# codebits1001/CET-driven-simulation-for-3D-printing-AM-KMC-Approach

Measured on AMD Instinct MI355X. Metric: kmc_events_per_sec, higher is better.
Workload: dtype f64

## Files before the change

cet-driven-simulation-for-3d-printing-am-kmc-approach_amd/cetkmc/_lib.py:

```python
import ctypes as C
import glob
import os
import subprocess

_HERE = os.path.dirname(os.path.abspath(__file__))
CSRC = os.path.join(os.path.dirname(_HERE), "csrc")
INCLUDE = os.path.join(os.path.dirname(os.path.dirname(_HERE)), "include")
SO_PATH = os.path.join(CSRC, "libcetkmc_hip.so")


def sources():
    return sorted(glob.glob(os.path.join(CSRC, "*.hip")) + glob.glob(os.path.join(CSRC, "*.hpp")) +
                  glob.glob(os.path.join(INCLUDE, "*.h")))


HIPCC_FLAGS = ["--offload-arch=gfx950", "-O3", "-std=c++17", "-fPIC", "-shared", "-ffp-contract=off",
               "-fno-fast-math", "-I/opt/rocm/include"]


class Params(C.Structure):
    _fields_ = [
        ("nu", C.c_double), ("nu_dep", C.c_double), ("E_b", C.c_double * 3), ("E_diff", C.c_double * 3),
        ("kT", C.c_double), ("T_melt", C.c_double), ("I0", C.c_double), ("delta_T_c", C.c_double),
        ("K_nuc", C.c_double), ("beta_imp_nuc", C.c_double), ("max_imp_frac", C.c_double),
# ... 20 lines not shown
        ("np_cap", C.c_int64), ("rng_mode", C.c_int32), ("seed", C.c_uint64), ("thermal_mode", C.c_int32),
        ("thermal_dt", C.c_double), ("q_planes", C.POINTER(C.c_double)), ("n_q", C.c_int64),
        ("use_latent", C.c_int32), ("profile", C.c_int32), ("incremental", C.c_int32),
    ]


class SuperArgs(C.Structure):
    _fields_ = [
        ("step0", C.c_int64), ("n_steps", C.c_int64), ("box", C.c_int32), ("defect_fraction", C.c_double),
        ("seed", C.c_uint64), ("thermal_mode", C.c_int32), ("thermal_dt", C.c_double),
        ("q_planes", C.POINTER(C.c_double)), ("n_q", C.c_int64), ("use_latent", C.c_int32), ("null_events", C.c_int32),
    ]


class LocalArgs(C.Structure):
    _fields_ = [
        ("step0", C.c_int64), ("n_steps", C.c_int64), ("box", C.c_int32), ("defect_fraction", C.c_double),
        ("seed", C.c_uint64), ("thermal_mode", C.c_int32), ("thermal_dt", C.c_double), ("max_events", C.c_int32),
        ("horizon_events", C.c_double),
    ]


class LaneTableInfo(C.Structure):
    _fields_ = [(n, C.c_int64) for n in ("fresh", "chunks", "usable", "poisoned", "builds")]


class Counters(C.Structure):
    _fields_ = [(n, C.c_int64) for n in ("steps", "sweeps", "incremental_steps", "thermal_updates", "supersteps", "bytes_h2d",
                                         "bytes_d2h", "alg_bytes_sweep", "alg_bytes_thermal", "profiled_steps")] + \
               [(n, C.c_double) for n in ("ms_thermal", "ms_interface", "ms_sweep", "ms_dirty_rows", "ms_reduce", "ms_select_apply")] + \
               [(n, C.c_int64) for n in ("alg_bytes_table", "table_updates", "interface_launches")] + \
               [("ms_comm", C.c_double), ("comm_calls", C.c_int64), ("deferred_steps", C.c_int64),
                ("early_tiles", C.c_int64)]


ALLGATHER_FN = C.CFUNCTYPE(C.c_int, C.c_void_p, C.c_void_p, C.c_void_p, C.c_int64)
EXCHANGE_FN = C.CFUNCTYPE(C.c_int, C.c_void_p, C.c_int, C.c_int, C.c_void_p, C.c_void_p, C.c_void_p, C.c_void_p, C.c_int64)


class HostComm(C.Structure):
    _fields_ = [("allgather", ALLGATHER_FN), ("exchange", EXCHANGE_FN), ("user", C.c_void_p)]


class RunResult(C.Structure):
    _fields_ = [
        ("steps_done", C.c_int64), ("status", C.c_int32), ("np_used", C.c_int64), ("q_used", C.c_int64),
        ("nucleation_count", C.c_int64), ("sweep_ms_total", C.c_double), ("sweep_launches", C.c_int64),
# ... 97 lines not shown
STRUCT_MIRRORS = {"params": Params, "event": Event, "sweep_info": SweepInfo, "run_args": RunArgs, "run_result": RunResult,
                  "super_args": SuperArgs, "counters": Counters, "host_comm": HostComm, "ens_args": EnsArgs,
                  "ens_analysis": EnsAnalysis, "front_stats": FrontStats, "layer_rec": LayerRec,
                  "texture_args": TextureArgs, "grain_rec": GrainRec, "solid_info": SolidInfo, "solid_args": SolidArgs,
                  "solid_rec": SolidRec, "origin_rec": OriginRec, "local_args": LocalArgs,
                  "remelt_info": RemeltInfo, "substep_info": SubstepInfo, "implicit_info": ImplicitInfo,
                  "thermal_boundary": ThermalBoundary, "boundary_info": BoundaryInfo,
                  "beam": Beam, "beam_info": BeamInfo}

_P = C.POINTER
PROTOTYPES = {
    "cetkmc_last_error": (C.c_char_p, []),
    "cetkmc_abi_version": (C.c_int, []),
    "cetkmc_source_hash": (C.c_char_p, []),
    "cetkmc_struct_size": (C.c_int, [C.c_char_p]),
    "cetkmc_dirty_offset": (C.c_int, [C.c_int, C.c_int]),
    "cetkmc_stale_row": (C.c_int, [C.c_int, _P(C.c_int), _P(C.c_int), C.c_int, C.c_int]),
    "cetkmc_stale_rows": (C.c_int, [C.c_int, _P(C.c_int), _P(C.c_int), C.c_int, C.c_void_p]),
    "cetkmc_table_tile_of": (C.c_int, [C.c_int, C.c_int, C.c_int]),
    "cetkmc_early_tile_row": (C.c_int, [C.c_int, C.c_int, C.c_int, C.c_int]),
    "cetkmc_lane_needs_values": (C.c_int, [C.c_uint64]),
    "cetkmc_lane_request": (C.c_int, [C.c_uint64, C.c_int]),
    "cetkmc_lane_table": (C.c_int, [C.c_void_p, _P(LaneTableInfo)]),
    "cetkmc_invalidates": (C.c_int, [C.c_char_p]),
    "cetkmc_device_count": (C.c_int, [_P(C.c_int)]),
    "cetkmc_create": (C.c_int, [_P(Params), C.c_int, C.c_int, _P(C.c_int), _P(C.c_void_p)]),
    "cetkmc_get_unique_id": (C.c_int, [C.c_char_p]),
    "cetkmc_create_rank": (C.c_int, [_P(Params), C.c_int, C.c_int, C.c_int, C.c_int, C.c_char_p, _P(C.c_void_p)]),
    "cetkmc_create_rank_host": (C.c_int, [_P(Params), C.c_int, C.c_int, C.c_int, C.c_int, _P(HostComm), _P(C.c_void_p)]),
    "cetkmc_destroy": (C.c_int, [C.c_void_p]),
    "cetkmc_set_params": (C.c_int, [C.c_void_p, _P(Params)]),
    "cetkmc_sync": (C.c_int, [C.c_void_p]),
    "cetkmc_set_option": (C.c_int, [C.c_void_p, C.c_char_p, C.c_int64]),
    "cetkmc_owned_planes": (C.c_int, [C.c_void_p, _P(C.c_int), _P(C.c_int)]),
    "cetkmc_upload": (C.c_int, [C.c_void_p, C.c_void_p, C.c_void_p, C.c_void_p, C.c_void_p, C.c_void_p]),
    "cetkmc_download": (C.c_int, [C.c_void_p, C.c_void_p, C.c_void_p, C.c_void_p, C.c_void_p, C.c_void_p]),
    "cetkmc_upload_planes": (C.c_int, [C.c_void_p, C.c_int, C.c_int, C.c_void_p, C.c_void_p, C.c_void_p, C.c_void_p, C.c_void_p]),
    "cetkmc_download_planes": (C.c_int, [C.c_void_p, C.c_int, C.c_int, C.c_void_p, C.c_void_p, C.c_void_p, C.c_void_p, C.c_void_p]),
    "cetkmc_set_defects": (C.c_int, [C.c_void_p, C.c_void_p]),
    "cetkmc_set_prev_state": (C.c_int, [C.c_void_p, C.c_void_p]),
    "cetkmc_thermal_cet": (C.c_int, [C.c_void_p, C.c_double, C.c_int]),
    "cetkmc_thermal_laser": (C.c_int, [C.c_void_p, C.c_double, C.c_void_p, C.c_int, C.c_int]),
    "cetkmc_rate_sweep": (C.c_int, [C.c_void_p, _P(SweepInfo)]),
    "cetkmc_select": (C.c_int, [C.c_void_p, C.c_double, _P(Event)]),
    "cetkmc_apply": (C.c_int, [C.c_void_p, _P(Event), C.c_double, C.c_double, C.c_int]),
    "cetkmc_enumerate_events": (C.c_int, [C.c_void_p, C.c_void_p, C.c_int64, _P(C.c_int64)]),
# ... 169 lines not shown
```

cet-driven-simulation-for-3d-printing-am-kmc-approach_amd/cetkmc/engine.py:

```python
import ctypes as C

import numpy as np

from . import _lib
from ._lib import Counters, EnsAnalysis, EnsArgs, Event, LaneTableInfo, LocalArgs, Params, RunArgs, RunResult, SuperArgs, SweepInfo, build_library

EVENT_DTYPE = np.dtype([("type", "<i4"), ("pos", "<i4", 3), ("target", "<i4", 3), ("atom", "<i4"),
                        ("rate", "<f8"), ("dep_rank", "<i8"), ("theta", "<f8"), ("phi", "<f8")], align=True)
assert EVENT_DTYPE.itemsize == C.sizeof(Event) == 64
FRONT_DTYPE = np.dtype([("n_front", "<i8"), ("n_skipped", "<i8"), ("pos_sum", "<i8", 3), ("G_sum", "<f8"), ("G_min", "<f8"),
                        ("G_max", "<f8"), ("Gi_sum", "<f8"), ("T_sum", "<f8"), ("n_melt", "<i8"), ("melt_bbox", "<i4", 6)],
                       align=True)
assert FRONT_DTYPE.itemsize == C.sizeof(_lib.FrontStats) == 112
LAYER_DTYPE = np.dtype([("n_occ", "<i8"), ("n_start", "<i8"), ("n_eq", "<i8"), ("seg", "<i8", 3), ("cut", "<i8", 3),
                        ("occ_state", "<i8", 4), ("gb_state", "<i8", 4), ("pad", "<i8")])
assert LAYER_DTYPE.itemsize == C.sizeof(_lib.LayerRec) == 144
GRAIN_DTYPE = np.dtype([("n", "<i8"), ("sum", "<i8", 3), ("sq", "<i8", 6), ("n_state", "<i8", 4), ("nb", "<i8", 4),
                        ("first_theta", "<f8"), ("first_phi", "<f8")])
assert GRAIN_DTYPE.itemsize == C.sizeof(_lib.GrainRec) == 160
SOLID_DTYPE = np.dtype([("n_rec", "<i8"), ("n_bad", "<i8"), ("n_cooling", "<i8"), ("stamp_sum", "<i8"), ("stamp_min", "<i8"),
                        ("stamp_max", "<i8"), ("q", "<i8", 4)])
assert SOLID_DTYPE.itemsize == C.sizeof(_lib.SolidRec) == 80
SOLID_INFO_DTYPE = np.dtype([("n_new", "<i8"), ("n_cleared", "<i8"), ("n_recorded", "<i8")])
assert SOLID_INFO_DTYPE.itemsize == C.sizeof(_lib.SolidInfo) == 24
# ... 431 lines not shown
        res = RunResult()
        totals = np.zeros(n + 1, np.float64) if want_logs else None
        events = np.zeros(max(n, 1), dtype=EVENT_DTYPE) if want_logs else None
        nev = np.zeros(max(n, 1), np.int64) if want_logs else None
        self._ck(self.lib.cetkmc_run_steps(self.h, C.byref(a), C.byref(res), _ptr(totals), _ptr(events), _ptr(nev)))
        done = res.steps_done
        out = dict(done=int(done), status=int(res.status), np_used=int(res.np_used), q_used=int(res.q_used),
                   nucleation_count=int(res.nucleation_count), sweep_ms_total=res.sweep_ms_total,
                   sweep_launches=int(res.sweep_launches), wall_ms=res.wall_ms, full_sweeps=int(res.full_sweeps),
                   min_margin=float(res.min_margin))
        if want_logs:
            out.update(totals=totals[:done + (1 if res.status == 1 else 0)], events=events[:done], n_events=nev[:done])
        return out

    def counters(self, reset=False):
        c = Counters()
        self._ck(self.lib.cetkmc_get_counters(self.h, C.byref(c), int(bool(reset))))
        return {n: getattr(c, n) for n, _ in Counters._fields_}

    def lane_table(self):
        info = LaneTableInfo()
        self._ck(self.lib.cetkmc_lane_table(self.h, C.byref(info)))
        return {n: int(getattr(info, n)) for n, _ in LaneTableInfo._fields_}

    def run_supersteps(self, step0, n, box, defect_fraction, seed, thermal_mode=1, thermal_dt=1e-6, q_planes=None,
                       use_latent=True, want_events=False, null_events=False):
        a = SuperArgs()
        q = None if q_planes is None else np.ascontiguousarray(q_planes, dtype=np.float64)
        a.step0, a.n_steps, a.box, a.defect_fraction, a.seed = int(step0), int(n), int(box), float(defect_fraction), int(seed)
        a.thermal_mode, a.thermal_dt = int(thermal_mode), float(thermal_dt)
        a.q_planes, a.n_q, a.use_latent = _dptr(q), (0 if q is None else q.shape[0]), int(bool(use_latent))
        a.null_events = int(bool(null_events))
        nbx = self.L // int(box) if box and self.L % int(box) == 0 else 1
        D = max(1, (self.i1 - self.i0) // int(box)) * nbx * nbx if box and self.L % int(box) == 0 else 1
        return self._supersteps(self.lib.cetkmc_run_supersteps, a, n, D, (D,) if want_events else None)

    def _supersteps(self, call, a, n, D, event_shape, more=()):
        res = RunResult()
        totals = np.zeros(n + 1, np.float64)
        n_exec = np.zeros(max(n, 1), np.int64)
        dt_event = np.zeros(max(n, 1), np.float64)
        events = None if event_shape is None else np.zeros((max(n, 1),) + event_shape, dtype=EVENT_DTYPE)
        logs = {name: np.zeros(max(n, 1), dtype) for name, dtype in more}
        self._ck(call(self.h, C.byref(a), C.byref(res), _ptr(totals), _ptr(events), _ptr(n_exec), _ptr(dt_event),
                      *[_ptr(v) for v in logs.values()]))
        done = int(res.steps_done)
# ... 495 lines not shown
```

cet-driven-simulation-for-3d-printing-am-kmc-approach_amd/csrc/cetkmc_hip.hip:

```cpp
#include <dlfcn.h>
#include <hip/hip_runtime.h>
#include <hip/hip_ext.h>
#include <rccl/rccl.h>

#include <algorithm>
#include <chrono>
#include <cmath>
#include <cstdint>
#include <climits>
#include <cstdio>
#include <cstring>
#include <map>
#include <mutex>
#include <string>
#include <type_traits>
#include <vector>

#include "kernels.hpp"
#include "cluster.hpp"
#include "superstep.hpp"
#include "local.hpp"
#include "ensemble.hpp"
#include "front.hpp"
#include "layer.hpp"
// ... 125 lines not shown
    KParams kp{};
    int L = 0, Pk = 1, PB = 1, RJ = 0, pitchS = 0, pitchT = 0, pitchC = 0;
    int dev = 0;
    hipStream_t stream = nullptr, stream2 = nullptr;
    std::vector<Slab> slabs;
    SlabView* d_views[4] = {nullptr, nullptr, nullptr, nullptr};
    int cur = 0;
    int row_par = 0;
    int G = 1, my_first = 0;
    int own_i0 = 0, own_i1 = 0;
    BlockEnt* d_blocks = nullptr;
    cetkmc_event* d_events_all = nullptr;
    StepState* d_ss = nullptr;
    int* d_dirty = nullptr;
    PendRec* d_pend = nullptr;
    int apply_in_sweep = 1;
    int fused_tiles = 1;
    int table_lane_skip = 1;
    int lane_sums = 1;
    int early_tiles = -1;
    int early_blocks = 256;
    int poison_alt_rows = 0;
    bool pend_live = false;
    int64_t cnt_lane_builds = 0;
    int pend_early = 0;
    BatchCfg pend_cfg{};
    double* d_ktab = nullptr;
    KParams* d_kp = nullptr;
    void* d_scratch = nullptr;
    size_t scratch_bytes = 0;
    int* d_flag = nullptr;
    double* d_qtop = nullptr;
    double *d_u_pick = nullptr, *d_u_defect = nullptr, *d_u_np = nullptr, *d_q = nullptr, *d_log_total = nullptr;
    cetkmc_event* d_log_event = nullptr;
    int64_t* d_log_nev = nullptr;
    size_t cap_steps = 0, cap_np = 0, cap_q = 0;
    char* pin_in = nullptr; size_t pin_in_cap = 0;
    char* pin_out = nullptr; size_t pin_out_cap = 0;
    struct { bool valid = false, has_defect = false; int64_t step0 = 0, n_steps = 0, np_cap = 0, n_q = 0; int thermal_mode = 0; } staged;
    ncclComm_t comm = nullptr;
    int rank = 0, nranks = 1;
    bool swept = false;
    int sweep_auto = 1;
    int sweep_variant = 1;
    bool table_fresh = false;
    bool ifc_fresh = false;
    bool lanes_fresh = false;
// ... 504 lines not shown
    h->table_fresh = true;
    invalidate(h, Cause::table_written);
    return 0;
}

StreamArgs stream_args(Handle* h, const SlabView& v)
{
    StreamArgs sa{};
    sa.T_melt = h->kp.T_melt; sa.delta_T_c = h->kp.delta_T_c; sa.kT = h->kp.kT; sa.I0 = h->kp.I0;
    sa.rate_threshold = h->kp.rate_threshold; sa.K0 = host_k_eff(h->p, 0, 0);
    sa.L = v.L; sa.gi0 = v.gi0; sa.nloc = v.nloc; sa.RJ = v.RJ; sa.pitchC = v.pitchC; sa.pitchT = v.pitchT; sa.Pk = v.Pk;
    sa.cls = v.cls; sa.T = v.T; sa.vval = v.vval; sa.dep_val = v.dep_val; sa.rowsum = v.rowsum; sa.rowcnt = v.rowcnt;
    sa.lanesum = v.lanesum; sa.lanecnt = v.lanecnt;
    sa.group_first = 0; sa.group_count = (v.nloc + STREAM_NI - 1) / STREAM_NI;
    return sa;
}

TableCfg table_cfg(Handle* h, const Slab& s, int par)
{
    TableCfg tb{};
    tb.T_melt = h->kp.T_melt; tb.delta_T_c = h->kp.delta_T_c; tb.kT = h->kp.kT; tb.I0 = h->kp.I0;
    tb.rate_threshold = h->kp.rate_threshold; tb.K0 = host_k_eff(h->p, 0, 0); tb.nu_dep = h->kp.nu_dep;
    tb.vval = s.vvalbuf[par]; tb.dep_val = s.depbuf[par];
    return tb;
}

int refresh_ifc_grid(Handle* h)
{
    for (auto& sl : h->slabs) {
        int n_list = 0;
        HIPCHK(hipMemcpy(&n_list, sl.v.ifc_n, sizeof(int), hipMemcpyDeviceToHost));
        grow_ifc_grid(h, n_list);
    }
    return 0;
}

inline bool multi_rank(const Handle* h) { return h->comm != nullptr || h->hc.allgather != nullptr; }
int one_slab_only(const Handle* h, const std::string& who, const char* why)
{
    if (h->slabs.size() != 1 || h->nranks != 1 || multi_rank(h)) return fail(who + " needs the whole lattice in one slab of one process" + why);
    return 0;
}
int thermal_exclusions(const ThermalSettings& s, const char* fn)
{
    const struct { bool on; const char *what, *setter, *mode_b, *ahead; } rows[] = {
        {s.remelt_on != 0, "remelting is on", "cetkmc_set_remelt", "Mode B has no melt", "the field computed ahead knows no melt"},
// ... 102 lines not shown
        if (sv == 4) {
            with_rows(rs, [&](auto hw, auto ch2) {
                launch(k_sweep_plane<hw.value, ch2.value>, dim3((unsigned)v.nloc), dim3(1024), plane_shmem(h->L), h->stream, xa, xb, sa, ss, h->d_blocks);
            });
        } else if (sv == 3) {
            const int ipp = rs.hw ? (h->L + 1) / 2 : h->L;
            const int64_t n_items = (int64_t)ipp * v.nloc;
            const dim3 g((unsigned)((n_items + 4 * TABLE_IPW - 1) / (4 * TABLE_IPW)));
            with_rows(rs, [&](auto hw, auto ch2) {
                launch(k_sweep_table<hw.value, ch2.value>, g, dim3(256), 0, h->stream, xa, xb, sa, ss);
            });
        } else if (h->sweep_variant >= 1 && h->pend_live) {
            ApplyArgs X{h->kp, (const SlabView*)dviews(h), h->d_pend, h->d_ss, h->pend_cfg, (const double*)h->d_u_defect,
                        (const double*)h->d_u_np, (const double*)h->d_ktab, h->d_log_total, h->d_log_event, h->d_log_nev};
            if (table_tiles(h, 1))
                with_flag(h->table_lane_skip != 0, [&](auto ls) {
                    with_flag(lane_table_use(h), [&](auto lu) {
                        const int late = table_tile_count(h->L, v.nloc, true) - h->pend_early;
                        launch(k_sweep_stream_apply<true, 1, false, true, ls.value, ls.value && lu.value>, dim3(late + 1), dim3(256), apply_shmem(), h->stream, xa, xb, sa, h->d_ss, X, h->pend_early);
                    });
                });
            else
                launch(k_sweep_stream_apply<true, 1, false>, dim3(sa.group_count * njt + 1), dim3(256), h->shmem_stream, h->stream, xa, xb, sa, h->d_ss, X, 0);
        } else if (h->sweep_variant == 1 && table_tiles(h, 2)) {
            const bool build = lane_table_on(h) && !h->lanes_fresh;
            with_flag(h->table_lane_skip != 0, [&](auto ls) {
                with_flag(build, [&](auto lb) {
                    launch(k_sweep_stream<true, true, 1, false, true, ls.value, lb.value>, dim3(table_tile_count(h->L, v.nloc, true)), dim3(256), 0, h->stream, xa, xb, sa, ss);
                });
            });
            if (build) { h->lanes_fresh = true; ++h->cnt_lane_builds; }
        } else if (h->sweep_variant >= 1) {
            auto go = [&](auto k) { launch(k, dim3(sa.group_count * njt), dim3(256), h->shmem_stream, h->stream, xa, xb, sa, ss); };
            if (h->sweep_variant == 1 && lane_table_on(h) && !h->lanes_fresh) {
                go(k_sweep_stream<true, true, 1, false, false, false, true>);
                h->lanes_fresh = true; ++h->cnt_lane_builds;
            }
            else if (h->sweep_variant == 1) with_stream_kernel<true>(rs, go); else with_stream_kernel<false>(rs, go);
        } else {
            hipLaunchKernelGGL(k_sweep_simple, dim3(v.nloc * njt), dim3(256), shmem0, h->stream, h->kp, v, h->d_ktab, ss);
        }
    }
    if (ev_b && !ext) HIPCHK(hipEventRecord(ev_b, h->stream));
    if (sv != 4)
        for (size_t s = 0; s < h->slabs.size(); ++s) {
            SlabView v = view_of(h, (int)s);
// ... 119 lines not shown
    if (multi_rank(h) && h->nranks > 1) {
        Slab& s = h->slabs[0];
        double* T = s.Tbuf[buf];
        CHK(comm_exchange(h, T + plane * 2, T, T + plane * s.v.nloc, T + plane * (s.v.nloc + 2), 2 * plane * 8));
    }
    return 0;
}

ThermalCfg thermal_cfg(Handle* h, double dt, int laser, int use_latent, int scrub)
{
    ThermalCfg C{};
    C.dt = dt; C.alpha = h->p.alpha; C.inv_dx2 = h->p.inv_dx2; C.clip_lo = h->p.T_clip_lo; C.clip_hi = h->p.T_clip_hi;
    C.T_nan = h->p.T_nan; C.rho_cp = h->p.rho_cp; C.latent_coef = h->p.latent_coef;
    C.laser = laser; C.use_latent = use_latent; C.scrub = scrub; C.ni = h->therm_ni;
    return C;
}

int launch_thermal_one(Handle* h, double dt, int laser, const double* d_q, int use_latent, int scrub, bool batch, bool first = true)
{
    const ThermalCfg C = thermal_cfg(h, dt, laser, use_latent, scrub);
    if (first) ++h->cnt.thermal_updates;
    for (auto& sl : h->slabs) h->cnt.alg_bytes_thermal += (int64_t)16 * sl.v.nloc * h->L * h->L;
    const int nxt = h->cur ^ 1;
    size_t n_fused = 0;
    const StepState* ssp = batch ? h->d_ss : nullptr;
    for (size_t s = 0; s < h->slabs.size(); ++s) {
        SlabView v = view_of(h, (int)s);
        const double* Tin = h->slabs[s].Tbuf[h->cur];
        double* Tout = h->slabs[s].Tbuf[nxt];
        uint8_t* prev = h->slabs[s].prev;
        if (h->thermal_variant == 1) {
            const dim3 grid = thermal_grid(h->L, v.nloc, h->therm_ni);
            if (h->L % THERM_KT == 0 && h->L % THERM16_TJ == 0 && !h->thermal_general && h->thermal_tiles16) {
                ThermalCfg C16 = C;
                C16.ni = h->therm_ni16;
                const dim3 g16(h->L / h->thermal_kt, h->L / THERM16_TJ, (v.nloc + C16.ni - 1) / C16.ni);
                const bool fuse = h->thermal_table && h->thermal_rpt == 2 && h->thermal_kt == 256 && h->sweep_variant >= 1;
                if (fuse) { ++n_fused; h->cnt.alg_bytes_table += (int64_t)8 * v.nloc * v.L * v.L; }
                with_source(laser, use_latent, [&](auto la, auto lt) {
                    auto go = [&](auto k, unsigned threads, const TableCfg& tb) {
                        launch(k, g16, dim3(threads), 0, h->stream, nullptr, nullptr, v, Tin, Tout, prev, d_q, C16, ssp, tb);
                    };
                    if (fuse) go(k_thermal_tiles16<la.value, lt.value, 2, 256, true>, 1024, table_cfg(h, h->slabs[s], nxt));
                    else if (h->thermal_rpt == 2 && h->thermal_kt == 128) go(k_thermal_tiles16<la.value, lt.value, 2, 128>, 512, TableCfg{});
                    else if (h->thermal_rpt == 2) go(k_thermal_tiles16<la.value, lt.value, 2, 256>, 1024, TableCfg{});
                    else go(k_thermal_tiles16<la.value, lt.value, 4, 256>, 512, TableCfg{});
                });
            } else if (h->L % THERM_KT == 0 && h->L % THERM_TJ == 0 && !h->thermal_general) {
                with_source(laser, use_latent, [&](auto la, auto lt) {
                    launch(k_thermal_tiles<la.value, lt.value>, grid, dim3(256), 0, h->stream, nullptr, nullptr, v, Tin, Tout, prev, d_q, C, ssp);
                });
            } else {
                hipLaunchKernelGGL(k_thermal_march, grid, dim3(256), 0, h->stream, v, Tin, Tout, prev, d_q, C, ssp);
            }
        } else {
            hipLaunchKernelGGL(k_thermal, dim3((h->L + 255) / 256, h->L, v.nloc), dim3(256), 0, h->stream, v, Tin, Tout,
                               (const uint8_t*)prev, d_q, C, ssp);
        }
    }
    HIPCHK(hipGetLastError());
    CHK(exchange_T_halo(h, nxt));
    if (laser && use_latent) {
        for (auto& s : h->slabs) {
            if (h->thermal_variant != 1)
                HIPCHK(hipMemcpyAsync(s.prev, s.v.state, s.nS, hipMemcpyDeviceToDevice, h->stream));
            hipLaunchKernelGGL(k_clear_row_flags, dim3(64), dim3(256), 0, h->stream, s.v, batch ? (const StepState*)h->d_ss : nullptr);
        }
        HIPCHK(hipGetLastError());
    }
    h->cur = nxt;
    const bool wrote_table = n_fused == h->slabs.size();
    invalidate(h, wrote_table ? Cause::thermal_update_wrote_table : Cause::thermal_update);
    if (wrote_table) { h->table_fresh = true; ++h->cnt.table_updates; }
    return 0;
}

int substep_block_of(const Handle* h)
{
    if (h->slabs.size() != 1 || multi_rank(h) || h->thermal_variant != 1) return 1;
    if (h->substep_block) return h->substep_block;
    return h->L > SUB_PLAIN_L ? SUB_SDEFAULT : 1;
}
int substep_planes_of(Handle* h, int S)
{
    if (h->substep_planes) return h->substep_planes;
    if (!h->n_cu && hipDeviceGetAttribute(&h->n_cu, hipDeviceAttributeMultiprocessorCount, h->dev) != hipSuccess) { (void)hipGetLastError(); h->n_cu = 256; }
    const int tiles = ((h->L + SUB_EK - 2 * S - 1) / (SUB_EK - 2 * S)) * ((h->L + SUB_EJ - 2 * S - 1) / (SUB_EJ - 2 * S));
    const int groups = std::max(1, h->n_cu / tiles), nloc = h->slabs[0].v.nloc;
    return std::max((nloc + groups - 1) / groups, std::min(nloc, 8));
}
template <int LASER, int S>
void launch_sub_S(Handle* h, const SlabView& v, const double* Tin, double* Tout, const double* d_q, const ThermalCfg& C, const StepState* ssp)
{
    const dim3 grid((h->L + SUB_EK - 2 * S - 1) / (SUB_EK - 2 * S), (h->L + SUB_EJ - 2 * S - 1) / (SUB_EJ - 2 * S), (v.nloc + C.ni - 1) / C.ni);
    launch(k_thermal_sub<LASER, S>, grid, dim3(SUB_THREADS), 0, h->stream, nullptr, nullptr, v, Tin, Tout, d_q, C, ssp);
}
// ... 563 lines not shown
    se.type = type; se.pi = pos[0]; se.pj = pos[1]; se.ti = target[0]; se.tj = target[1];
    return se;
}
int cetkmc_stale_row(int type, const int pos[2], const int target[2], int gi, int j)
{
    return stale_row(stale_ev_host(type, pos, target), gi, j) ? 1 : 0;
}
int cetkmc_lane_needs_values(uint64_t class8)
{
    return lane_needs_values(make_uint2((unsigned)class8, (unsigned)(class8 >> 32))) ? 1 : 0;
}
int cetkmc_lane_request(uint64_t class8, int count_byte)
{
    static_assert(LANE_REQ_NONE == CETKMC_LANE_REQ_NONE && LANE_REQ_VALUES == CETKMC_LANE_REQ_VALUES && LANE_REQ_SUM == CETKMC_LANE_REQ_SUM, "cetkmc.h");
    return lane_request(make_uint2((unsigned)class8, (unsigned)(class8 >> 32)), (unsigned)count_byte & 0xFFu);
}
int cetkmc_lane_table(void* handle, cetkmc_lane_table_info* out)
{
    Handle* h = (Handle*)handle;
    if (!h || !out) return fail("null argument");
    *out = cetkmc_lane_table_info{};
    out->fresh = lane_table_use(h) ? 1 : 0;
    out->builds = h->cnt_lane_builds;
    if (h->slabs.size() != 1 || !h->slabs[0].v.lanecnt) return 0;
    HIPCHK(hipSetDevice(h->dev));
    CHK(ensure_scratch(h, 2 * sizeof(unsigned long long)));
    unsigned long long* d = (unsigned long long*)h->d_scratch;
    unsigned long long got[2] = {0, 0};
    HIPCHK(hipMemsetAsync(d, 0, sizeof got, h->stream));
    hipLaunchKernelGGL(k_lane_census, dim3(256), dim3(256), 0, h->stream, h->slabs[0].v, d);
    HIPCHK(hipGetLastError());
    HIPCHK(hipMemcpyAsync(got, d, sizeof got, hipMemcpyDeviceToHost, h->stream));
    HIPCHK(hipStreamSynchronize(h->stream));
    out->chunks = (int64_t)h->slabs[0].v.nloc * h->L * (h->pitchT / 8);
    out->usable = (int64_t)got[0];
    out->poisoned = (int64_t)got[1];
    return 0;
}
int cetkmc_table_tile_of(int L, int gi, int j)
{
    if (L <= 128 || L > 256 || gi < 0 || gi >= L || j < 0 || j >= L) return -1;
    return table_tile_of(L, true, gi, j);
}
int cetkmc_early_tile_row(int L, int early_tiles, int gi, int j)
{
    const int t = cetkmc_table_tile_of(L, gi, j);
    return t < 0 ? -1 : (t < early_tiles ? 1 : 0);
}
int cetkmc_stale_rows(int type, const int pos[2], const int target[2], int L, int rows[][2])
{
    const StaleEv se = stale_ev_host(type, pos, target);
    int n = 0;
    for (int c = 0; c < STALE_CAND; ++c) {
        int gi, j;
        if (!stale_candidate(se, L, c, gi, j)) continue;
        if (n < PATCH_MAX) { rows[n][0] = gi; rows[n][1] = j; }
        ++n;
    }
    return n;
}
// ... 129 lines not shown
    if (!strcmp(key, "substep_block")) {
        if (value < 0 || value > SUB_SMAX) return fail("substep_block must be 0 (default), 1 (plain path: one launch per sub-step) or 2.." + std::to_string(SUB_SMAX) + " sub-steps per k_thermal_sub launch");
        h->substep_block = (int)value;
        return 0;
    }
    if (!strcmp(key, "substep_planes")) {
        if (value < 0 || value > 4096) return fail("substep_planes must be 0 (default: one round of blocks) or 1..4096 planes per block of k_thermal_sub");
        h->substep_planes = (int)value;
        return 0;
    }
    if (!strcmp(key, "apply_in_sweep")) { h->apply_in_sweep = value ? 1 : 0; return 0; }
    if (!strcmp(key, "fused_tiles")) {
        if (value < 0 || value > 2) return fail("fused_tiles must be 0 (ring tiles), 1 (census-free tiles in the launch that applies a pending event, default) or 2 (in the plain streaming launch at that shape as well)");
        h->fused_tiles = (int)value;
        return 0;
    }
    if (!strcmp(key, "table_lane_skip")) { h->table_lane_skip = value ? 1 : 0; return 0; }
    if (!strcmp(key, "lane_sums")) {
        if (value < 0 || value > 1) return fail("lane_sums must be 0 (the tiles read table entries) or 1 (lane sums of pristine chunks, default)");
        h->lane_sums = (int)value;
        h->lanes_fresh = false;
        return 0;
    }
    if (!strcmp(key, "early_tiles")) {
        if (value < -1 || value > INT32_MAX) return fail("early_tiles must be a tile count >= 0, or -1 (a quarter of the tiles)");
        h->early_tiles = (int)value;
        return 0;
    }
    if (!strcmp(key, "early_blocks")) {
        if (value < 0 || value > INT32_MAX) return fail("early_blocks must be a block count >= 0");
        h->early_blocks = (int)value;
        return 0;
    }
    if (!strcmp(key, "poison_alt_rows")) { h->poison_alt_rows = value ? 1 : 0; return 0; }
    if (!strcmp(key, "thermal_table")) { h->thermal_table = value ? 1 : 0; return 0; }
    if (!strcmp(key, "reserve_batch")) {
        if (value < 0 || value > (1 << 22)) return fail("reserve_batch out of range");
        HIPCHK(hipSetDevice(h->dev));
        invalidate(h, Cause::option_reserve_batch);
        const size_t n = (size_t)value;
        CHK(reserve_steps(h, n));
        CHK(grow(&h->d_u_np, &h->cap_np, 2 * n + 2 + (size_t)h->L * h->L));
        CHK(grow(&h->d_q, &h->cap_q, (n / 20 + 2) * (size_t)h->L * h->L));
        CHK(grow_pinned(&h->pin_in, &h->pin_in_cap, 2 * n * 8 + (2 * n + 2) * 8 + std::min<size_t>(PIN_SMALL_MAX, (n / 20 + 2) * (size_t)h->L * h->L * 8)));
        CHK(grow_pinned(&h->pin_out, &h->pin_out_cap, 64 + n * (16 + sizeof(cetkmc_event)) + h->slabs.size() * sizeof(int) + (h->ts.remelt_on ? 8 + 4 * 8 : 0)));
        return reserve_events(h, std::max<int64_t>(7 * std::min<int64_t>(value, 256), value <= 64 ? 2 * value : 2 * (value / 8 + 1)));
// ... 2538 lines not shown
```

cet-driven-simulation-for-3d-printing-am-kmc-approach_amd/csrc/kernels.hpp:

```cpp
#pragma once
#include "voxel.hpp"
#include "../../include/cetkmc.h"

namespace cetkmc {

struct BlockEnt { double sum; int64_t cnt; };

struct StepState {
    int64_t cur;
    int32_t status;
    int32_t pad0;
    int64_t np_pos;
    int64_t nuc_count;
    double  total;
    int64_t n_events;
    int64_t n_dep;
    double  min_margin;
};

template <class S> __device__ __forceinline__ const auto& ens_rep(unsigned r, const S& sel) { return sel.reps[r]; }
template <class S> __device__ __forceinline__ int ens_rel(const S& sel) { return sel.rel; }
template <class S> __device__ __forceinline__ unsigned ens_nz(const S& sel) { return (unsigned)sel.nz; }
template <class S> __device__ __forceinline__ int64_t ens_stride(const S& sel) { return sel.stride; }
template <class S> __device__ __forceinline__ const long long* ens_offs(const S& sel) { return sel.offs; }
// ... 268 lines not shown
    int32_t* rowcnt;
    double* lanesum;
    uint8_t* lanecnt;
};

__device__ __forceinline__ double nuc_bulk(double T_melt, double delta_T_c, double kT, double I0, double thr, double K0, double Traw)
{
    const double Tc = pymax(Traw, 1.0);
    const double dT = T_melt - Tc;
    double r = 0.0;
    if (dT > delta_T_c) {
        r = nuc_rate_s(I0, K0, dT, kT * Tc);
        if (!(r > thr && finite_d(r))) r = 0.0;
    }
    return r;
}

__device__ __forceinline__ unsigned alignbyte(unsigned hi, unsigned lo, unsigned n) { return __builtin_amdgcn_alignbyte(hi, lo, n); }
__device__ __forceinline__ double mask_f64(double v, unsigned w, int b)
{
    const int m = __builtin_amdgcn_sbfe(w, b, 1);
    return __hiloint2double(__double2hiint(v) & m, __double2loint(v) & m);
}
__device__ __forceinline__ double tree8(const double (&x)[8])
{
    return ((x[0] + x[1]) + (x[2] + x[3])) + ((x[4] + x[5]) + (x[6] + x[7]));
}

template <bool TAB, bool HW>
__device__ __forceinline__ void load_vals(const StreamArgs& A, int li, int jrow, int lane, int m, double (&v)[8])
{
    const int k0 = min((m << 9) + 8 * (HW ? (lane & 31) : lane), A.pitchT - 8);
    const int jr = min(jrow, A.L - 1);
    const double2* src = reinterpret_cast<const double2*>((TAB ? A.vval : A.T) + ((int64_t)li * A.L + jr) * A.pitchT + k0);
#pragma unroll
    for (int q = 0; q < 4; ++q) { const double2 t = src[q]; v[2 * q] = t.x; v[2 * q + 1] = t.y; }
}
__device__ __forceinline__ uint2 load_cls8(const StreamArgs& A, int li, int jrow, int sl, int m)
{
    const int k0 = min((m << 9) + 8 * sl, A.pitchT - 8);
    const int jr = min(jrow, A.L - 1);
    return *reinterpret_cast<const uint2*>(A.cls + ((int64_t)li * A.RJ + (jr + 2)) * A.pitchC + KOFFC + k0);
}

constexpr int LM_NONE = 0, LM_BUILD = 1, LM_USE = 2;
__host__ __device__ __forceinline__ bool lane_pristine(uint2 own) { return own.x == 0x01010101u && own.y == 0x01010101u; }
__device__ __forceinline__ int64_t lane_chunk(const StreamArgs& A, int li, int jrow, int sl)
// ... 418 lines not shown
            while (jp >= ipp) { jp -= ipp; ++lp; }
        }
        return;
    }
    table_item_request<HW>(A, lp, jrow_of(jp), lane, va, ca);
    auto step = [&](double (&cur)[8], uint2& ccur, double (&nxt)[8], uint2& cnxt, bool last) {
        int lp2 = lp, jp2 = jp + 4;
        while (jp2 >= ipp) { jp2 -= ipp; ++lp2; }
        const bool more = !last && (item + 4 < n_items);
        const int lpn = more ? lp2 : lp, jpn = more ? jp2 : jp;
        table_item_request<HW>(A, lpn, jrow_of(jpn), lane, nxt, cnxt);
        table_item_reduce<HW, CH2, SK, LM>(A, lp, jrow_of(jp), lane, cur, ccur, sw);
        item += 4; lp = lp2; jp = jp2;
    };
#pragma unroll 1
    for (int t = 0; t < IPW; t += 2) {
        step(va, ca, vb, cb, false);
        if (item >= n_items) break;
        step(vb, cb, va, ca, t + 2 >= IPW);
        if (item >= n_items) break;
    }
}

template <bool TAB, bool HW, int NPF, bool CH2, bool TT = false, bool LS = false, bool LB = false>
__global__ __launch_bounds__(256) CETKMC_SWEEP_ATTR void k_sweep_stream(StreamArgs A, const StepState* __restrict__ ss)
{
    static_assert(!TT || TAB, "census-free tiles read the rate table");
    static_assert(!LS || TT, "lanes are skipped by the census-free tiles");
    constexpr int LM = LB ? LM_BUILD : LM_NONE;
    if (ss && ss->status) return;
    if constexpr (TT) {
        sweep_table_tile<HW, CH2, false, TABLE_TILE_IPW, LS, LM>(A, blockIdx.x, (int)gridDim.x);
    } else {
        extern __shared__ __attribute__((aligned(16))) unsigned char smem[];
        sweep_stream_tile<TAB, HW, NPF, CH2, false, LM>(A, blockIdx.x, smem);
    }
}

template <bool HW, bool CH2>
__global__ __launch_bounds__(256) CETKMC_SWEEP_ATTR void k_sweep_table(StreamArgs A, const StepState* __restrict__ ss)
{
    if (ss && ss->status) return;
    sweep_table_tile<HW, CH2, false, TABLE_IPW>(A, blockIdx.x, (int)gridDim.x);
}

__global__ __launch_bounds__(256) void k_lane_census(SlabView S, unsigned long long* out)
{
    const int cpr = S.pitchT >> 3;
    const int64_t n = (int64_t)S.nloc * S.L * cpr, first = (int64_t)2 * S.L * cpr;
    int ok = 0, bad = 0;
    for (int64_t q = (int64_t)blockIdx.x * blockDim.x + threadIdx.x; q < n; q += (int64_t)gridDim.x * blockDim.x) {
        const unsigned c = S.lanecnt[first + q];
// ... 1099 lines not shown
}

__global__ void k_empty() {}

template <class... E>
__global__ void k_batch_reset(StepState* ss, E... ens)
{
    if constexpr (sizeof...(E) > 0) {
        const auto& e = ens_rep(blockIdx.x, ens...);
        ss = e.ss;
        if (!e.active) { ss->cur = 0; ss->status = 1; ss->np_pos = 0; ss->min_margin = 1.0; return; }
    }
    ss->cur = 0; ss->status = 0; ss->np_pos = 0; ss->min_margin = 1.0;
}

struct ThermalCfg {
    double dt, alpha, inv_dx2, clip_lo, clip_hi, T_nan, rho_cp, latent_coef;
    int laser, use_latent, scrub, ni;
};
struct TableCfg {
    double T_melt, delta_T_c, kT, I0, rate_threshold, K0, nu_dep;
    double* vval;
    double* dep_val;
};
__device__ __forceinline__ double scrub_T(double x, double T_nan, int on)
{
    if (!on) return x;
    if (x != x) return T_nan;
    if (__builtin_isinf(x)) return x > 0 ? 1.7976931348623157e308 : -1.7976931348623157e308;
    return x;
}
__global__ __launch_bounds__(256) void k_thermal(SlabView S, const double* __restrict__ Tin, double* __restrict__ Tout,
                                                 const uint8_t* __restrict__ prev_state, const double* __restrict__ q_top,
                                                 ThermalCfg C, const StepState* __restrict__ ss)
{
    const int L = S.L;
    const int k = blockIdx.x * blockDim.x + threadIdx.x;
    const int j = blockIdx.y, lp = blockIdx.z;
    if (k >= L) return;
    const int li = lp + 2, i = S.gi0 + lp;
    const int64_t c = S.tidx(li, j, k);
    if (ss && ss->status) { Tout[c] = Tin[c]; return; }
    const int im = (i > 0 ? i - 1 : 0) - (S.gi0 - 2), ip = (i < L - 1 ? i + 1 : L - 1) - (S.gi0 - 2);
    const int jm = j > 0 ? j - 1 : 0, jp = j < L - 1 ? j + 1 : L - 1;
    const int km = k > 0 ? k - 1 : 0, kp = k < L - 1 ? k + 1 : L - 1;
    const double tc = scrub_T(Tin[c], C.T_nan, C.scrub);
    const double d0 = tc * -2.0 + (scrub_T(Tin[S.tidx(im, j, k)], C.T_nan, C.scrub) + scrub_T(Tin[S.tidx(ip, j, k)], C.T_nan, C.scrub));
// ... 299 lines not shown
                        qterm = (qv != 0.0) ? qv / C.rho_cp : 0.0;
                    }
                    double dF = 0.0;
                    if (LATENT && ((pv2 >> (8 * h)) & 255u) == 0 && ((st2 >> (8 * h)) & 255u) != 0) dF = 1.0 / dtm;
                    const double dTdt = C.alpha * lap + qterm + C.latent_coef * dF;
                    nt = tc + C.dt * dTdt;
                }
                double v = nt < C.clip_lo ? C.clip_lo : nt;
                out[h] = v > C.clip_hi ? C.clip_hi : v;
            }
            *reinterpret_cast<double2*>(Tout + (int64_t)li * pstride + off[q]) = make_double2(out[0], out[1]);
        }
        __syncthreads();
#pragma unroll
        for (int q = 0; q < 4; ++q) { prv[q][0] = cur[q][0]; prv[q][1] = cur[q][1]; cur[q][0] = nxt[q][0]; cur[q][1] = nxt[q][1]; }
        rt = rt_n; rb = rb_n; rs = rs_n;
    }
}

constexpr int THERM16_TJ = 16, THERM16_NI = 16;
#ifndef CETKMC_THERM16_ATTR
#define CETKMC_THERM16_ATTR __attribute__((amdgpu_waves_per_eu(4, 4)))
#endif
template <bool LASER, bool LATENT, int RPT, int KT, bool TABLE = false>
__global__ __launch_bounds__((KT / 2) * (16 / RPT)) CETKMC_THERM16_ATTR void k_thermal_tiles16(SlabView S, const double* __restrict__ Tin, double* __restrict__ Tout,
                                                         uint8_t* __restrict__ prev_state, const double* __restrict__ q_top,
                                                         ThermalCfg C, const StepState* __restrict__ ss, TableCfg TB = TableCfg{})
{
    constexpr int TJ = THERM16_TJ, LW = KT + 2, HC = KT / 2, NTHR = HC * (16 / RPT);
    static_assert(NTHR >= 2 * KT, "one rim cell per thread");
    __shared__ double tile[(TJ + 2) * LW];
    const int L = S.L, pitchT = S.pitchT;
    const int tid = threadIdx.x;
    const int kc = blockIdx.x * KT, j0 = blockIdx.y * TJ;
    const int lp0 = blockIdx.z * C.ni, lp1 = min(lp0 + C.ni, S.nloc);
    constexpr int RS = TJ / RPT;
    const int col = 2 * (tid % HC), rbase = tid / HC;
    const int k0 = kc + col;
    const int64_t pstride = (int64_t)L * pitchT;
    int off[RPT];
#pragma unroll
    for (int q = 0; q < RPT; ++q) off[q] = (j0 + rbase + RS * q) * pitchT + k0;
    if (ss && ss->status) {
        for (int lp = lp0; lp < lp1; ++lp)
#pragma unroll
            for (int q = 0; q < RPT; ++q) {
                const int64_t c = (int64_t)(lp + 2) * pstride + off[q];
                *reinterpret_cast<double2*>(Tout + c) = *reinterpret_cast<const double2*>(Tin + c);
            }
        return;
    }
    const int scrub = C.scrub;
    auto lplane = [&](int i) { return (i < 0 ? 0 : (i > L - 1 ? L - 1 : i)) - (S.gi0 - 2); };
// ... 67 lines not shown
                const double lap = ((d0 + d1) + d2) * C.inv_dx2;
                double nt;
                if (!LASER) {
                    nt = tc + dt_alpha * lap;
                } else {
                    double qterm = 0.0;
                    if (top) {
                        const double qv = q_top[(int64_t)j * L + k0 + h];
                        qterm = (qv != 0.0) ? qv / C.rho_cp : 0.0;
                    }
                    double dF = 0.0;
                    if (LATENT && ((pv2 >> (8 * h)) & 255u) == 0 && ((st2 >> (8 * h)) & 255u) != 0) dF = 1.0 / dtm;
                    const double dTdt = C.alpha * lap + qterm + C.latent_coef * dF;
                    nt = tc + C.dt * dTdt;
                }
                double v = nt < C.clip_lo ? C.clip_lo : nt;
                out[h] = v > C.clip_hi ? C.clip_hi : v;
            }
            *reinterpret_cast<double2*>(Tout + (int64_t)li * pstride + off[q]) = make_double2(out[0], out[1]);
            if (TABLE) {
                const double r0 = nuc_bulk(TB.T_melt, TB.delta_T_c, TB.kT, TB.I0, TB.rate_threshold, TB.K0, out[0]);
                const double r1 = nuc_bulk(TB.T_melt, TB.delta_T_c, TB.kT, TB.I0, TB.rate_threshold, TB.K0, out[1]);
                *reinterpret_cast<double2*>(TB.vval + (int64_t)li * pstride + off[q]) = make_double2(r0, r1);
                if (i == L - 1) {
                    double* dp = TB.dep_val + (int64_t)j * pitchT + k0;
                    dp[0] = dep_rate_s(TB.nu_dep, TB.T_melt, TB.kT, pymax(out[0], 1.0));
                    dp[1] = dep_rate_s(TB.nu_dep, TB.T_melt, TB.kT, pymax(out[1], 1.0));
                }
            }
        }
        __syncthreads();
#pragma unroll
        for (int q = 0; q < RPT; ++q) {
            prv[q][0] = cur[q][0]; prv[q][1] = cur[q][1]; cur[q][0] = nxt[q][0]; cur[q][1] = nxt[q][1];
            nxt[q][0] = nx2[q][0]; nxt[q][1] = nx2[q][1];
        }
        rr = rr_n; rs = rs_n;
    }
}

template <class SRC>
__global__ void k_pack_u8(SlabView S, uint8_t* dst, const SRC* __restrict__ src, int i_begin, int nplanes, int with_cls)
{
    const int L = S.L;
    const int64_t n = (int64_t)nplanes * L * L;
    for (int64_t idx = (int64_t)blockIdx.x * blockDim.x + threadIdx.x; idx < n; idx += (int64_t)gridDim.x * blockDim.x) {
// ... 68 lines not shown
```

include/cetkmc.h:

```cpp
#ifndef CETKMC_H
#define CETKMC_H

#include <stdint.h>

#ifdef __cplusplus
extern "C" {
#endif

#define CETKMC_ABI_VERSION 1

typedef struct cetkmc_params {
    double nu;
    double nu_dep;
    double E_b[3];
    double E_diff[3];
    double kT;
    double T_melt;
    double I0;
    double delta_T_c;
    double K_nuc;
    double beta_imp_nuc;
    double max_imp_frac;
    double rate_threshold;
    double anisotropy;
// ... 84 lines not shown
    int64_t profiled_steps;
    double  ms_thermal, ms_interface , ms_sweep, ms_dirty_rows, ms_reduce, ms_select_apply;
    int64_t alg_bytes_table;
    int64_t table_updates;
    int64_t interface_launches;
    double  ms_comm;
    int64_t comm_calls;
    int64_t deferred_steps;
    int64_t early_tiles;
} cetkmc_counters;

const char* cetkmc_last_error(void);
int cetkmc_abi_version(void);
const char* cetkmc_source_hash(void);
int cetkmc_struct_size(const char* name);
int cetkmc_dirty_offset(int di, int dj);
int cetkmc_stale_row(int type, const int pos[2], const int target[2], int gi, int j);
int cetkmc_stale_rows(int type, const int pos[2], const int target[2], int L, int rows[][2]);
int cetkmc_table_tile_of(int L, int gi, int j);
int cetkmc_early_tile_row(int L, int early_tiles, int gi, int j);
int cetkmc_lane_needs_values(uint64_t class8);
enum cetkmc_lane_req { CETKMC_LANE_REQ_NONE = 0, CETKMC_LANE_REQ_VALUES = 1, CETKMC_LANE_REQ_SUM = 2 };
int cetkmc_lane_request(uint64_t class8, int count_byte);
typedef struct cetkmc_lane_table_info { int64_t fresh, chunks, usable, poisoned, builds; } cetkmc_lane_table_info;
int cetkmc_lane_table(void* handle, cetkmc_lane_table_info* out);
enum cetkmc_cache {
    CETKMC_CACHE_SWEEP = 1,
    CETKMC_CACHE_TABLE = 2,
    CETKMC_CACHE_IFC = 4,
    CETKMC_CACHE_APPLIED = 8,
    CETKMC_CACHE_STAGED = 16
};
int cetkmc_invalidates(const char* cause);
int cetkmc_device_count(int* n);

int cetkmc_create(const cetkmc_params* p, int L, int n_slabs, const int* device_ids, void** handle);
int cetkmc_get_unique_id(char out[128]);
int cetkmc_create_rank(const cetkmc_params* p, int L, int rank, int nranks, int device_id,
                       const char unique_id[128], void** handle);
typedef int (*cetkmc_allgather_fn)(void* user, const void* send, void* recv, int64_t nbytes);
typedef int (*cetkmc_exchange_fn)(void* user, int lo, int hi, const void* send_lo, void* recv_lo, const void* send_hi,
                                  void* recv_hi, int64_t nbytes);
typedef struct cetkmc_host_comm {
    cetkmc_allgather_fn allgather;
    cetkmc_exchange_fn exchange;
    void* user;
} cetkmc_host_comm;
int cetkmc_create_rank_host(const cetkmc_params* p, int L, int rank, int nranks, int device_id, const cetkmc_host_comm* hc,
// ... 237 lines not shown
```

Before: 20130.

## Build lane sum table inside fused thermal kernel and let sweep reuse it

New measurement: 20620 (median of 6 runs). 1.02x the previous value.

```diff
diff --git a/cet-driven-simulation-for-3d-printing-am-kmc-approach_amd/cetkmc/_lib.py b/cet-driven-simulation-for-3d-printing-am-kmc-approach_amd/cetkmc/_lib.py
--- a/cet-driven-simulation-for-3d-printing-am-kmc-approach_amd/cetkmc/_lib.py
+++ b/cet-driven-simulation-for-3d-printing-am-kmc-approach_amd/cetkmc/_lib.py
@@ -66,7 +66,7 @@
 
 
 class LaneTableInfo(C.Structure):
-    _fields_ = [(n, C.c_int64) for n in ("fresh", "chunks", "usable", "poisoned", "builds")]
+    _fields_ = [(n, C.c_int64) for n in ("fresh", "chunks", "usable", "poisoned", "builds", "builds_thermal")]
 
 
 class Counters(C.Structure):
@@ -210,6 +210,9 @@
     "cetkmc_lane_needs_values": (C.c_int, [C.c_uint64]),
     "cetkmc_lane_request": (C.c_int, [C.c_uint64, C.c_int]),
     "cetkmc_lane_table": (C.c_int, [C.c_void_p, _P(LaneTableInfo)]),
+    "cetkmc_lane_table_copy": (C.c_int, [C.c_void_p, C.c_void_p, C.c_void_p, C.c_int64]),
+    "cetkmc_lane_quad_node": (None, [_P(C.c_double), C.c_int, _P(C.c_double), _P(C.c_int)]),
+    "cetkmc_tree8": (C.c_double, [_P(C.c_double)]),
     "cetkmc_invalidates": (C.c_int, [C.c_char_p]),
     "cetkmc_device_count": (C.c_int, [_P(C.c_int)]),
     "cetkmc_create": (C.c_int, [_P(Params), C.c_int, C.c_int, _P(C.c_int), _P(C.c_void_p)]),
diff --git a/cet-driven-simulation-for-3d-printing-am-kmc-approach_amd/cetkmc/engine.py b/cet-driven-simulation-for-3d-printing-am-kmc-approach_amd/cetkmc/engine.py
--- a/cet-driven-simulation-for-3d-printing-am-kmc-approach_amd/cetkmc/engine.py
+++ b/cet-driven-simulation-for-3d-printing-am-kmc-approach_amd/cetkmc/engine.py
@@ -477,6 +477,13 @@
         info = LaneTableInfo()
         self._ck(self.lib.cetkmc_lane_table(self.h, C.byref(info)))
         return {n: int(getattr(info, n)) for n, _ in LaneTableInfo._fields_}
+
+    def lane_table_arrays(self):
+        n = self.lane_table()["chunks"]
+        sums, counts = np.empty(n, np.float64), np.empty(n, np.uint8)
+        self._ck(self.lib.cetkmc_lane_table_copy(self.h, sums.ctypes.data, counts.ctypes.data, n))
+        shape = (self.i1 - self.i0, self.L, n // ((self.i1 - self.i0) * self.L))
+        return sums.reshape(shape), counts.reshape(shape)
 
     def run_supersteps(self, step0, n, box, defect_fraction, seed, thermal_mode=1, thermal_dt=1e-6, q_planes=None,
                        use_latent=True, want_events=False, null_events=False):
diff --git a/cet-driven-simulation-for-3d-printing-am-kmc-approach_amd/csrc/cetkmc_hip.hip b/cet-driven-simulation-for-3d-printing-am-kmc-approach_amd/csrc/cetkmc_hip.hip
--- a/cet-driven-simulation-for-3d-printing-am-kmc-approach_amd/csrc/cetkmc_hip.hip
+++ b/cet-driven-simulation-for-3d-printing-am-kmc-approach_amd/csrc/cetkmc_hip.hip
@@ -171,7 +171,10 @@
     int early_blocks = 256;
     int poison_alt_rows = 0;
     bool pend_live = false;
+    int lane_build = 1;
+    int lane_sweep = 1;
     int64_t cnt_lane_builds = 0;
+    int64_t cnt_lane_builds_thermal = 0;
     int pend_early = 0;
     BatchCfg pend_cfg{};
     double* d_ktab = nullptr;
@@ -722,6 +725,7 @@
     tb.T_melt = h->kp.T_melt; tb.delta_T_c = h->kp.delta_T_c; tb.kT = h->kp.kT; tb.I0 = h->kp.I0;
     tb.rate_threshold = h->kp.rate_threshold; tb.K0 = host_k_eff(h->p, 0, 0); tb.nu_dep = h->kp.nu_dep;
     tb.vval = s.vvalbuf[par]; tb.dep_val = s.depbuf[par];
+    tb.lanesum = s.v.lanesum; tb.lanecnt = s.v.lanecnt;
     return tb;
 }
 
@@ -870,6 +874,8 @@
                 });
             else
                 launch(k_sweep_stream_apply<true, 1, false>, dim3(sa.group_count * njt + 1), dim3(256), h->shmem_stream, h->stream, xa, xb, sa, h->d_ss, X, 0);
+        } else if (h->lane_sweep && lane_table_use(h)) {
+            launch(k_sweep_stream<true, true, 1, false, true, true, false, true>, dim3(table_tile_count(h->L, v.nloc, true)), dim3(256), 0, h->stream, xa, xb, sa, ss);
         } else if (h->sweep_variant == 1 && table_tiles(h, 2)) {
             const bool build = lane_table_on(h) && !h->lanes_fresh;
             with_flag(h->table_lane_skip != 0, [&](auto ls) {
@@ -1035,7 +1041,7 @@
     if (first) ++h->cnt.thermal_updates;
     for (auto& sl : h->slabs) h->cnt.alg_bytes_thermal += (int64_t)16 * sl.v.nloc * h->L * h->L;
     const int nxt = h->cur ^ 1;
-    size_t n_fused = 0;
+    size_t n_fused = 0, n_lanes = 0;
     const StepState* ssp = batch ? h->d_ss : nullptr;
     for (size_t s = 0; s < h->slabs.size(); ++s) {
         SlabView v = view_of(h, (int)s);
@@ -1050,11 +1056,14 @@
                 const dim3 g16(h->L / h->thermal_kt, h->L / THERM16_TJ, (v.nloc + C16.ni - 1) / C16.ni);
                 const bool fuse = h->thermal_table && h->thermal_rpt == 2 && h->thermal_kt == 256 && h->sweep_variant >= 1;
                 if (fuse) { ++n_fused; h->cnt.alg_bytes_table += (int64_t)8 * v.nloc * v.L * v.L; }
+                const bool lanes = fuse && h->lane_build && lane_table_on(h);
+                if (lanes) { ++n_lanes; h->cnt.alg_bytes_table += (int64_t)9 * v.nloc * v.L * (v.pitchT / 8); }
                 with_source(laser, use_latent, [&](auto la, auto lt) {
                     auto go = [&](auto k, unsigned threads, const TableCfg& tb) {
                         launch(k, g16, dim3(threads), 0, h->stream, nullptr, nullptr, v, Tin, Tout, prev, d_q, C16, ssp, tb);
                     };
-                    if (fuse) go(k_thermal_tiles16<la.value, lt.value, 2, 256, true>, 1024, table_cfg(h, h->slabs[s], nxt));
+                    if (lanes) go(k_thermal_tiles16<la.value, lt.value, 2, 256, true, true>, 1024, table_cfg(h, h->slabs[s], nxt));
+                    else if (fuse) go(k_thermal_tiles16<la.value, lt.value, 2, 256, true>, 1024, table_cfg(h, h->slabs[s], nxt));
                     else if (h->thermal_rpt == 2 && h->thermal_kt == 128) go(k_thermal_tiles16<la.value, lt.value, 2, 128>, 512, TableCfg{});
                     else if (h->thermal_rpt == 2) go(k_thermal_tiles16<la.value, lt.value, 2, 256>, 1024, TableCfg{});
                     else go(k_thermal_tiles16<la.value, lt.value, 4, 256>, 512, TableCfg{});
@@ -1085,6 +1094,7 @@
     const bool wrote_table = n_fused == h->slabs.size();
     invalidate(h, wrote_table ? Cause::thermal_update_wrote_table : Cause::thermal_update);
     if (wrote_table) { h->table_fresh = true; ++h->cnt.table_updates; }
+    if (wrote_table && n_lanes == h->slabs.size()) { h->lanes_fresh = true; ++h->cnt_lane_builds_thermal; }
     return 0;
 }
 
@@ -1694,6 +1704,7 @@
     *out = cetkmc_lane_table_info{};
     out->fresh = lane_table_use(h) ? 1 : 0;
     out->builds = h->cnt_lane_builds;
+    out->builds_thermal = h->cnt_lane_builds_thermal;
     if (h->slabs.size() != 1 || !h->slabs[0].v.lanecnt) return 0;
     HIPCHK(hipSetDevice(h->dev));
     CHK(ensure_scratch(h, 2 * sizeof(unsigned long long)));
@@ -1708,6 +1719,32 @@
     out->usable = (int64_t)got[0];
     out->poisoned = (int64_t)got[1];
     return 0;
+}
+int cetkmc_lane_table_copy(void* handle, double* sums, uint8_t* counts, int64_t n)
+{
+    Handle* h = (Handle*)handle;
+    if (!h || !sums || !counts) return fail("null argument");
+    if (h->slabs.size() != 1 || !h->slabs[0].v.lanecnt) return fail("cetkmc_lane_table_copy: the shape has no lane table");
+    const SlabView& v = h->slabs[0].v;
+    const int64_t cpr = h->pitchT / 8, owned = (int64_t)v.nloc * h->L * cpr, first = (int64_t)2 * h->L * cpr;
+    if (n != owned) return fail("cetkmc_lane_table_copy: n must be the owned chunks, " + std::to_string(owned));
+    HIPCHK(hipSetDevice(h->dev));
+    HIPCHK(hipMemcpyAsync(sums, v.lanesum + first, (size_t)n * sizeof(double), hipMemcpyDeviceToHost, h->stream));
+    HIPCHK(hipMemcpyAsync(counts, v.lanecnt + first, (size_t)n, hipMemcpyDeviceToHost, h->stream));
+    HIPCHK(hipStreamSynchronize(h->stream));
+    return 0;
+}
+void cetkmc_lane_quad_node(const double* x8, int lane, double* sum, int* count)
+{
+    double x[8];
+    for (int q = 0; q < 8; ++q) x[q] = x8[q];
+    lane_quad_node(x, lane, *sum, *count);
+}
+double cetkmc_tree8(const double* x8)
+{
+    double x[8];
+    for (int q = 0; q < 8; ++q) x[q] = x8[q];
+    return tree8(x);
 }
 int cetkmc_table_tile_of(int L, int gi, int j)
 {
@@ -1883,6 +1920,8 @@
         h->lanes_fresh = false;
         return 0;
     }
+    if (!strcmp(key, "lane_build")) { h->lane_build = value ? 1 : 0; return 0; }
+    if (!strcmp(key, "lane_sweep")) { h->lane_sweep = value ? 1 : 0; return 0; }
     if (!strcmp(key, "early_tiles")) {
         if (value < -1 || value > INT32_MAX) return fail("early_tiles must be a tile count >= 0, or -1 (a quarter of the tiles)");
         h->early_tiles = (int)value;
diff --git a/cet-driven-simulation-for-3d-printing-am-kmc-approach_amd/csrc/kernels.hpp b/cet-driven-simulation-for-3d-printing-am-kmc-approach_amd/csrc/kernels.hpp
--- a/cet-driven-simulation-for-3d-printing-am-kmc-approach_amd/csrc/kernels.hpp
+++ b/cet-driven-simulation-for-3d-printing-am-kmc-approach_amd/csrc/kernels.hpp
@@ -314,7 +314,7 @@
     const int m = __builtin_amdgcn_sbfe(w, b, 1);
     return __hiloint2double(__double2hiint(v) & m, __double2loint(v) & m);
 }
-__device__ __forceinline__ double tree8(const double (&x)[8])
+__host__ __device__ __forceinline__ double tree8(const double (&x)[8])
 {
     return ((x[0] + x[1]) + (x[2] + x[3])) + ((x[4] + x[5]) + (x[6] + x[7]));
 }
@@ -779,12 +779,13 @@
     }
 }
 
-template <bool TAB, bool HW, int NPF, bool CH2, bool TT = false, bool LS = false, bool LB = false>
+template <bool TAB, bool HW, int NPF, bool CH2, bool TT = false, bool LS = false, bool LB = false, bool LU = false>
 __global__ __launch_bounds__(256) CETKMC_SWEEP_ATTR void k_sweep_stream(StreamArgs A, const StepState* __restrict__ ss)
 {
     static_assert(!TT || TAB, "census-free tiles read the rate table");
     static_assert(!LS || TT, "lanes are skipped by the census-free tiles");
-    constexpr int LM = LB ? LM_BUILD : LM_NONE;
+    static_assert(!LU || (LS && !LB), "lane sums are read by the skipping tiles of a launch that does not build them");
+    constexpr int LM = LB ? LM_BUILD : LU ? LM_USE : LM_NONE;
     if (ss && ss->status) return;
     if constexpr (TT) {
         sweep_table_tile<HW, CH2, false, TABLE_TILE_IPW, LS, LM>(A, blockIdx.x, (int)gridDim.x);
@@ -1930,7 +1931,18 @@
     double T_melt, delta_T_c, kT, I0, rate_threshold, K0, nu_dep;
     double* vval;
     double* dep_val;
+    double* lanesum;
+    uint8_t* lanecnt;
 };
+__host__ __device__ inline void lane_quad_node(const double (&x)[8], int l, double& sum, int& cnt)
+{
+    double p[4], q[4];
+    int np[4], nq[4];
+    for (int a = 0; a < 4; ++a) { p[a] = x[2 * a] + x[2 * a + 1]; np[a] = (x[2 * a] != 0.0 ? 1 : 0) + (x[2 * a + 1] != 0.0 ? 1 : 0); }
+    for (int a = 0; a < 4; ++a) { q[a] = p[a] + p[a ^ 1]; nq[a] = np[a] + np[a ^ 1]; }
+    sum = q[l & 3] + q[(l & 3) ^ 2];
+    cnt = nq[l & 3] + nq[(l & 3) ^ 2];
+}
 __device__ __forceinline__ double scrub_T(double x, double T_nan, int on)
 {
     if (!on) return x;
@@ -2276,13 +2288,14 @@
 #ifndef CETKMC_THERM16_ATTR
 #define CETKMC_THERM16_ATTR __attribute__((amdgpu_waves_per_eu(4, 4)))
 #endif
-template <bool LASER, bool LATENT, int RPT, int KT, bool TABLE = false>
+template <bool LASER, bool LATENT, int RPT, int KT, bool TABLE = false, bool LANES = false>
 __global__ __launch_bounds__((KT / 2) * (16 / RPT)) CETKMC_THERM16_ATTR void k_thermal_tiles16(SlabView S, const double* __restrict__ Tin, double* __restrict__ Tout,
                                                          uint8_t* __restrict__ prev_state, const double* __restrict__ q_top,
                                                          ThermalCfg C, const StepState* __restrict__ ss, TableCfg TB = TableCfg{})
 {
     constexpr int TJ = THERM16_TJ, LW = KT + 2, HC = KT / 2, NTHR = HC * (16 / RPT);
     static_assert(NTHR >= 2 * KT, "one rim cell per thread");
+    static_assert(!LANES || (TABLE && KT % 8 == 0 && HC % 4 == 0), "the lane table is stored with the table, a chunk per quad of lanes");
     __shared__ double tile[(TJ + 2) * LW];
     const int L = S.L, pitchT = S.pitchT;
     const int tid = threadIdx.x;
@@ -2396,6 +2409,19 @@
                 const double r0 = nuc_bulk(TB.T_melt, TB.delta_T_c, TB.kT, TB.I0, TB.rate_threshold, TB.K0, out[0]);
                 const double r1 = nuc_bulk(TB.T_melt, TB.delta_T_c, TB.kT, TB.I0, TB.rate_threshold, TB.K0, out[1]);
                 *reinterpret_cast<double2*>(TB.vval + (int64_t)li * pstride + off[q]) = make_double2(r0, r1);
+                if constexpr (LANES) {
+                    double s = r0 + r1;
+                    s = s + dpp_f64(s, 0);
+                    s = s + dpp_f64(s, 1);
+                    unsigned nz = (r0 != 0.0 ? 1u : 0u) + (r1 != 0.0 ? 1u : 0u);
+                    nz += __builtin_amdgcn_update_dpp(nz, nz, 0xB1, 0xF, 0xF, true);
+                    nz += __builtin_amdgcn_update_dpp(nz, nz, 0x4E, 0xF, 0xF, true);
+                    if ((tid & 3) == 0) {
+                        const int64_t ch = ((int64_t)li * pstride + off[q]) >> 3;
+                        TB.lanesum[ch] = s;
+                        TB.lanecnt[ch] = (uint8_t)nz;
+                    }
+                }
                 if (i == L - 1) {
                     double* dp = TB.dep_val + (int64_t)j * pitchT + k0;
                     dp[0] = dep_rate_s(TB.nu_dep, TB.T_melt, TB.kT, pymax(out[0], 1.0));
diff --git a/include/cetkmc.h b/include/cetkmc.h
--- a/include/cetkmc.h
+++ b/include/cetkmc.h
@@ -130,8 +130,11 @@
 int cetkmc_lane_needs_values(uint64_t class8);
 enum cetkmc_lane_req { CETKMC_LANE_REQ_NONE = 0, CETKMC_LANE_REQ_VALUES = 1, CETKMC_LANE_REQ_SUM = 2 };
 int cetkmc_lane_request(uint64_t class8, int count_byte);
-typedef struct cetkmc_lane_table_info { int64_t fresh, chunks, usable, poisoned, builds; } cetkmc_lane_table_info;
+typedef struct cetkmc_lane_table_info { int64_t fresh, chunks, usable, poisoned, builds, builds_thermal; } cetkmc_lane_table_info;
 int cetkmc_lane_table(void* handle, cetkmc_lane_table_info* out);
+int cetkmc_lane_table_copy(void* handle, double* sums, uint8_t* counts, int64_t n);
+void cetkmc_lane_quad_node(const double* x8, int lane, double* sum, int* count);
+double cetkmc_tree8(const double* x8);
 enum cetkmc_cache {
     CETKMC_CACHE_SWEEP = 1,
     CETKMC_CACHE_TABLE = 2,
```
